# zhaozijie2022/LocoTouch

Hardware: AMD Instinct MI355X
Metric: env-steps/sec (whole node), TransportTeacher 4096 envs/GPU (higher is better)
Workload: dtype f32

## Files before the change

locotouch_amd/_abi.py:

```python
from __future__ import annotations

import ctypes
import os
import re

_HERE = os.path.dirname(os.path.abspath(__file__))
REPO = os.path.dirname(_HERE)
LIB_PATH = os.environ.get("LOCOTOUCH_AMD_LIB", os.path.join(_HERE, "_lib", "liblocotouch_env.so"))

_SCALARS = {"int": ctypes.c_int, "int32_t": ctypes.c_int32, "int64_t": ctypes.c_int64, "uint8_t": ctypes.c_uint8,
            "uint32_t": ctypes.c_uint32, "uint64_t": ctypes.c_uint64, "size_t": ctypes.c_size_t, "float": ctypes.c_float,
            "double": ctypes.c_double}
_DECL = re.compile(r"(?:const\s+)?(\w+)\s*((?:\*\s*(?:const\b\s*)?)*)(\w*)\s*((?:\[[^\]]*\]\s*)*)")


def _ctype(decl, structs, opaque, consts, typed, param):
    m = _DECL.fullmatch(decl.strip())
    if not m:
        return None
    base, stars, name, dims = m.groups()
    depth = stars.count("*")
    try:
        dims = [sum(int(t) if t.strip().isdigit() else consts[t.strip()] for t in d.split("+")) for d in re.findall(r"\[([^\]]*)\]", dims)]
    except KeyError:
# ... 45 lines not shown
        if not m:
            if stmt == "}":
                continue
            raise ImportError(f"cannot parse declaration {stmt!r}")
        ret, name, args = m.groups()
        res = (None, None) if ret.strip() == "void" else _ctype(ret, structs, opaque, consts, typed, param=False)
        args = [] if args.strip() == "void" else [_ctype(a, structs, opaque, consts, typed, param=True) for a in args.split(",")]
        if res is None or None in args:
            raise ImportError(f"cannot type prototype {name}: {' '.join(stmt.split())!r}")
        protos[name] = (res[1], [t for _, t in args])
    return consts, structs, protos


class _CfgMethods(ctypes.Structure):
    def copy(self) -> "LtCfg":
        new = LtCfg()
        ctypes.memmove(ctypes.byref(new), ctypes.byref(self), ctypes.sizeof(self))
        for attr in ("extra_reward_terms", "extra_termination_terms", "extra_observation_terms", "reward_term_params"):
            if hasattr(self, attr):
                v = getattr(self, attr)
                setattr(new, attr, dict(v) if isinstance(v, dict) else list(v))
        return new

    def to_dict(self) -> dict:
        def py(v):
            return [py(x) for x in v] if hasattr(v, "__len__") else v

        return {name: py(getattr(self, name)) for name, *_ in self._fields_ if not name.startswith("_")}


_ENV_VALUE_QUERIES = (
    "lt_abi_version", "lt_cfg_sizeof", "lt_cfg_num_presets", "lt_cfg_preset_id", "lt_cfg_obs_dim", "lt_cfg_tactile_dim", "lt_last_error",
    "lt_wgrad_splits", "lt_wgrad_ws_floats", "lt_elu_backward_bias_ws_floats", "lt_head_wgrad_ws_floats", "lt_adam_clip_step_ws_floats",
    "lt_elu_backward_bias_nblk", "lt_head_wgrad_nblk", "lt_mlp_backward_blocks", "lt_env_kernel_name", "lt_mlp_kernel_name")

HEADERS = (
    ("", "lt_env.h", False, _ENV_VALUE_QUERIES, ("lt_cfg", "lt_view", "lt_mlp_desc", "lt_render_view", "lt_render_desc")),
    ("OBS_NORM", "lt_obs_norm.h", False, (), ()),
    ("STUDENT", "lt_student.h", True, ("lt_student_step_launches",), ("lt_student_desc", "lt_student_params")),
    ("COLLECT", "lt_collect.h", False, (), ()),
    ("LEDGER", "lt_ledger.h", False, (), ()),
    ("CNN_TRAIN", "lt_cnn_train.h", False, ("lt_cnn_launches",), ("lt_cnn_desc", "lt_cnn_params", "lt_cnn_grads")),
    ("BC", "lt_bc.h", False, (), ()),
    ("LSTM", "lt_lstm.h", False, (), ()),
    ("MEMORY", "lt_memory.h", False, (), ("lt_memory_net",)),
    ("MEMORY_SEQ", "lt_memory_seq.h", False, ("lt_memory_seq_backward_units",), ("lt_memory_seq_net", "lt_memory_seq_grad")),
    ("MEMORY_GRU", "lt_memory_gru.h", False, ("lt_memory_gru_seq_backward_units",),
     ("lt_memory_gru_net", "lt_memory_gru_seq_net", "lt_memory_gru_seq_grad")),
    ("POLICY", "lt_policy.h", True, ("lt_policy_step_launches",), ("lt_policy_desc", "lt_policy_memory")),
    ("PPO_OPTS", "lt_ppo_opts.h", False, (), ()),
    ("MLP_DX", "lt_mlp_dx.h", True, (), ()),
    ("PPO_SYM", "lt_ppo_sym.h", False, (), ()),
    ("ENCODER", "lt_encoder.h", False, ("lt_encoder_forward_launches",), ("lt_encoder_desc", "lt_encoder_net")),
)


def _bind(table, include_dir):
    bound, seen, env_structs = [], set(), None
    for prefix, fname, uses_env_structs, queries, _ in table:
        path, queries = os.path.join(include_dir, fname), frozenset(queries)
        consts, structs, sigs = parse_header(open(path).read(), structs=env_structs if uses_env_structs else None, bases={"lt_cfg": _CfgMethods})
        if not prefix:
            env_structs = structs
        for name in sorted(queries - set(sigs)):
            raise ImportError(f"include/{fname}: the value query {name} named in _abi.HEADERS is not declared there")
        for name, (restype, _) in sigs.items():
            if name in seen:
                raise ImportError(f"include/{fname}: {name} repeats an entry point of an earlier header")
            if restype is not ctypes.c_int and (prefix or name not in queries):
                raise ImportError(f"include/{fname}: {name} returns no int (a new value query of lt_env.h belongs in _abi.HEADERS)")
        seen.update(sigs)
        bound.append((path, consts, structs, sigs, queries))
    return bound


ALL_SIGNATURES: dict = {}
ALL_VALUE_QUERIES: set = set()
for (_prefix, _, _, _, _published), (_path, _consts, _structs, _sigs, _queries) in zip(HEADERS, _bind(HEADERS, os.path.join(REPO, "include"))):
    _p = _prefix + "_" if _prefix else ""
    globals().update(_consts)
    globals().update({_p + "HEADER": _path, _p + "CONSTS": _consts, _p + "SIGNATURES": _sigs, _p + "VALUE_QUERIES": _queries})
    globals().update({_structs[_c].__name__: _structs[_c] for _c in _published})
    if not _prefix:
        STRUCTS, EXPORTS = _structs, list(_sigs)
    ALL_SIGNATURES.update(_sigs)
    ALL_VALUE_QUERIES |= _queries

_lib = None
_calls: dict = {}


def load() -> ctypes.CDLL:
    global _lib
    if _lib is not None:
        return _lib
    if not os.path.exists(LIB_PATH):
        raise ImportError(f"{LIB_PATH} is missing: run `python -c 'import __graft_entry__ as g; g.build()'` "
                          "(the HIP extension is mandatory, there is no CPU fallback)")
    lib = ctypes.CDLL(LIB_PATH)
    for name, (restype, argtypes) in ALL_SIGNATURES.items():
        fn = getattr(lib, name)
        fn.restype, fn.argtypes = restype, argtypes
        if name not in ALL_VALUE_QUERIES:
            _calls[name] = (fn, [ptr if t is ctypes.c_void_p else _ref if issubclass(t, ctypes._Pointer) and issubclass(t._type_, ctypes.Structure)
                                 else None for t in argtypes])
    if lib.lt_cfg_sizeof() != ctypes.sizeof(LtCfg):
# ... 77 lines not shown
```

locotouch_amd/csrc/lt_ppo.hip:

```cpp
#include <hip/hip_runtime.h>
#include <math.h>
#include <stdint.h>

#include "lt_env.h"
#include "lt_host_check.h"
#include "lt_internal.h"
#include "lt_ppo_device.h"

namespace {

template <bool LOG, bool NORM>
__global__ __launch_bounds__(256) void lt_ppo_loss_kernel(const float* __restrict__ mu, const float* __restrict__ stdp, const float* __restrict__ value,
                                                          const float* __restrict__ actions, const float* __restrict__ old_logp,
                                                          const float* __restrict__ adv, const float* __restrict__ returns,
                                                          const float* __restrict__ old_values, const float* __restrict__ old_mu,
                                                          const float* __restrict__ old_sigma, const long long* __restrict__ idx,
                                                          long long M, int A, float clip, float vcoef, int clipped_value,
                                                          const float* __restrict__ adv_stats, float* __restrict__ dmu, float* __restrict__ dvalue, float* __restrict__ acc) {
  const long long row = (long long)blockIdx.x * 256 + threadIdx.x;
  const bool ok = row < M;
  const long long src = (ok && idx) ? idx[row] : row;
  __shared__ float sigma_lds[MAX_A];
  if constexpr (LOG) {
    if ((int)threadIdx.x < A) sigma_lds[threadIdx.x] = lt_sigma_of_log(stdp[threadIdx.x]);
    __syncthreads();
  }
  float part[4 + MAX_A];
  float amax_mu = 0.f, amax_v = 0.f;
#pragma unroll
  for (int i = 0; i < 4 + MAX_A; ++i) part[i] = 0.f;
  if (ok) {
    const float inv_m = 1.f / (float)M;
    float logp = 0.f, kl = 0.f;
    float z[MAX_A], isg[MAX_A];
#pragma unroll
    for (int a = 0; a < MAX_A; ++a) {
      if (a < A) {
        const float sg = LOG ? sigma_lds[a] : stdp[a], m = mu[row * A + a], x = actions[src * A + a];
        const float om = old_mu[src * A + a], os = old_sigma[src * A + a];
        isg[a] = 1.f / sg;
        z[a] = (x - m) * isg[a];
        logp += lt_ppo_logp_term<LOG>(z[a], sg, stdp[a]);
        kl += lt_ppo_kl_term(sg, os, om, m);
      }
    }
    float advr = adv[src];
    if constexpr (NORM) advr = (advr - adv_stats[0]) * adv_stats[1];
    const float ratio = __expf(logp - old_logp[src]);
    LT_PPO_SURROGATE(advr, ratio, clip, s1, s2, dsurr_dratio)
    const float dlogp = dsurr_dratio * ratio * inv_m;
#pragma unroll
    for (int a = 0; a < MAX_A; ++a) {
      if (a < A) {
        dmu[row * A + a] = dlogp * z[a] * isg[a];
        amax_mu = fmaxf(amax_mu, fabsf(dlogp * z[a] * isg[a]));
        if constexpr (LOG) part[4 + a] = dlogp * (z[a] * z[a] - 1.f);
        else part[4 + a] = dlogp * (z[a] * z[a] - 1.f) * isg[a];
      }
    }
    const float v = value[row], R = returns[src];
// ... 269 lines not shown
    p[i] = pi - step_size * (mi / (sqrtf(vi) / bc2_sqrt + eps));
  }
}

__global__ __launch_bounds__(64) void lt_std_from_log_kernel(const float* __restrict__ log_std, int A, float* __restrict__ stdp) {
  if ((int)threadIdx.x < A) stdp[threadIdx.x] = lt_sigma_of_log(log_std[threadIdx.x]);
}

__device__ __forceinline__ double lt_block_sum_f64(double v, double* red) {
#pragma unroll
  for (int off = 32; off > 0; off >>= 1) v += __shfl_xor(v, off, 64);
  __syncthreads();
  if ((threadIdx.x & 63) == 0) red[threadIdx.x >> 6] = v;
  __syncthreads();
  return (red[0] + red[1]) + (red[2] + red[3]);
}

__global__ __launch_bounds__(256) void lt_adv_stats_kernel(const float* __restrict__ adv, const long long* __restrict__ idx, long long M,
                                                           float* __restrict__ stats) {
#pragma clang fp reciprocal(off)
  __shared__ double red[4];
  const long long base = (long long)blockIdx.x * M;
  double s = 0.0;
  for (long long r = threadIdx.x; r < M; r += 256) s += (double)adv[idx ? idx[base + r] : base + r];
  const double mean = lt_block_sum_f64(s, red) / (double)M;
  double q = 0.0;
  for (long long r = threadIdx.x; r < M; r += 256) {
    const double d = (double)adv[idx ? idx[base + r] : base + r] - mean;
    q += d * d;
  }
  const double var = lt_block_sum_f64(q, red) / (double)(M - 1);
  if (threadIdx.x == 0) {
    stats[2 * blockIdx.x] = (float)mean;
    stats[2 * blockIdx.x + 1] = (float)(1.0 / (sqrt(var) + (double)1.0e-8f));
  }
}

__global__ __launch_bounds__(64) void lt_ppo_lr_rule_kernel(const float* __restrict__ kl_mean, float desired, float lr_min, float lr_max, float factor,
                                                            float* __restrict__ lr, float* __restrict__ stats, const float* __restrict__ scalars,
                                                            float* __restrict__ dstd_out, int A) {
  if (dstd_out && scalars && (int)threadIdx.x < A) dstd_out[threadIdx.x] = scalars[8 + threadIdx.x];
  if (threadIdx.x != 0) return;
  if (kl_mean && desired > 0.f) {
#pragma clang fp reciprocal(off)
    const float kl = *kl_mean;
    float v = *lr;
    if (kl > desired * 2.f) v = fmaxf(lr_min, v / factor);
    else if (kl < desired * 0.5f && kl > 0.f) v = fminf(lr_max, v * factor);
    *lr = v;
  }
  if (stats && scalars) { stats[0] += scalars[2]; stats[1] += scalars[1]; stats[2] += scalars[3]; }
}

}

extern "C" int lt_ppo_lr_rule(const float* kl_mean, float desired_kl, float lr_min, float lr_max, float factor, float* lr, float* stats,
                              const float* scalars, float* dstd_out, int num_actions, void* stream) {
  if (!lr || factor <= 1.f || num_actions < 0 || num_actions > MAX_A) return einval("lt_ppo_lr_rule: invalid argument");
  hipLaunchKernelGGL(lt_ppo_lr_rule_kernel, dim3(1), dim3(64), 0, (hipStream_t)stream, kl_mean, desired_kl, lr_min, lr_max, factor, lr, stats, scalars,
                     dstd_out, num_actions);
  return launch_status();
}

static int elu_backward_bias(const float* da, const float* a, int64_t M, int N, float alpha, float* dz, float* db, float* ws, float* amax, void* stream);
extern "C" int lt_elu_backward_bias(const float* da, const float* a, int64_t M, int N, float alpha, float* dz, float* db, float* ws, void* stream) {
  return elu_backward_bias(da, a, M, N, alpha, dz, db, ws, nullptr, stream);
}
extern "C" int lt_elu_backward_bias2(const float* da, const float* a, int64_t M, int N, float alpha, float* dz, float* db, float* ws, float* amax_blocks,
                                     void* stream) {
  return elu_backward_bias(da, a, M, N, alpha, dz, db, ws, amax_blocks, stream);
}
static int elu_backward_bias(const float* da, const float* a, int64_t M, int N, float alpha, float* dz, float* db, float* ws, float* amax, void* stream) {
  if (!da || !a || !dz || !ws || M < 1 || N < 4 || (N & 3) || N > 1024)
    return einval("lt_elu_backward_bias: invalid argument (N a multiple of 4, 4 <= N <= 1024)");
  const int nblk = (int)((M + EB_ROWS - 1) / EB_ROWS);
  hipLaunchKernelGGL(lt_elu_bwd_bias_kernel, dim3((unsigned)nblk), dim3(256), 0, (hipStream_t)stream, da, a, (long long)M, N, alpha, dz, ws, amax);
  if (db) launch_one_sum(ws, nblk, (long long)N, N, N, db, nullptr, (hipStream_t)stream);
  return launch_status();
}

extern "C" int64_t lt_head_wgrad_ws_floats(int64_t M, int n, int k) { return ((M + HW_ROWS - 1) / HW_ROWS) * ((int64_t)n * k + HW_MAX_N); }

extern "C" int lt_head_wgrad(const float* dy, const float* x, int x_split, int64_t M, int n, int k, float* dw, float* db, float* ws, void* stream) {
  if (!dy || !x || !ws || M < 1 || n < 1 || n > HW_MAX_N || k < 4 || (k & 3) || k > 1024)
    return einval("lt_head_wgrad: invalid argument (1 <= n <= 16, k a multiple of 4, 4 <= k <= 1024)");
  const int nblk = (int)((M + HW_ROWS - 1) / HW_ROWS), k4 = k / 4, lanes = 256 / k4;
  const int nn = n <= 1 ? 1 : (n <= 4 ? 4 : (n <= 8 ? 8 : (n <= 12 ? 12 : 16)));
  const size_t lds = (size_t)lanes * nn * k4 * 16 + (size_t)lanes * nn * 4;
  if (const int e = lt_ensure_dynamic_lds((const void*)lt_head_wgrad_kernel<16>, 72 * 1024)) {
    lt_set_error(hipGetErrorString((hipError_t)e));
    return LT_EHIP;
  }
  if (lds > 72 * 1024) return einval("lt_head_wgrad: n * k too large for one block's LDS partials");
  const dim3 g((unsigned)nblk), b(256);
  hipStream_t st = (hipStream_t)stream;
  switch (nn) {
    case 1: hipLaunchKernelGGL(lt_head_wgrad_kernel<1>, g, b, lds, st, dy, x, x_split, (long long)M, n, k, ws); break;
    case 4: hipLaunchKernelGGL(lt_head_wgrad_kernel<4>, g, b, lds, st, dy, x, x_split, (long long)M, n, k, ws); break;
    case 8: hipLaunchKernelGGL(lt_head_wgrad_kernel<8>, g, b, lds, st, dy, x, x_split, (long long)M, n, k, ws); break;
    case 12: hipLaunchKernelGGL(lt_head_wgrad_kernel<12>, g, b, lds, st, dy, x, x_split, (long long)M, n, k, ws); break;
    default: hipLaunchKernelGGL(lt_head_wgrad_kernel<16>, g, b, lds, st, dy, x, x_split, (long long)M, n, k, ws); break;
  }
  if (dw) launch_one_sum(ws, nblk, (long long)n * k + HW_MAX_N, n * k + n, n * k, dw, db, st);
  return launch_status();
}

// ... 77 lines not shown
                       std_is_log ? 1 : 0, out);
  return launch_status();
}

extern "C" int lt_ppo_loss(const float* mu, const float* stdp, const float* value, const float* actions, const float* old_logp, const float* adv,
                           const float* returns, const float* old_values, const float* old_mu, const float* old_sigma, const int64_t* idx,
                           int64_t M, int A, float clip, float value_loss_coef, float entropy_coef, int use_clipped_value_loss, float* dmu, float* dvalue,
                           float* acc, float* out, void* stream) {
  if (!mu || !stdp || !value || !actions || !old_logp || !adv || !returns || !old_values || !old_mu || !old_sigma || !dmu || !dvalue || !acc ||
      M < 1 || A < 1 || A > MAX_A)
    return einval("lt_ppo_loss: invalid argument (1 <= num_actions <= 16)");
  return ppo_loss(mu, stdp, value, actions, old_logp, adv, returns, old_values, old_mu, old_sigma, idx, M, A, clip, value_loss_coef,
                  entropy_coef, use_clipped_value_loss, 0, nullptr, dmu, dvalue, acc, out, stream);
}

extern "C" int lt_ppo_loss_opts(const float* mu, const float* stdp, const float* value, const float* actions, const float* old_logp,
                                const float* adv, const float* returns, const float* old_values, const float* old_mu, const float* old_sigma,
                                const int64_t* idx, int64_t M, int A, float clip, float value_loss_coef, float entropy_coef,
                                int use_clipped_value_loss, int std_is_log, const float* adv_stats, float* dmu, float* dvalue, float* acc,
                                float* out, void* stream) {
  const char* fn = "lt_ppo_loss_opts";
  const ptr_check ptrs[] = {{"mu", mu, 4}, {"std", stdp, 4}, {"value", value, 4}, {"actions", actions, 4}, {"old_logp", old_logp, 4}, {"adv", adv, 4},
                            {"returns", returns, 4}, {"old_values", old_values, 4}, {"old_mu", old_mu, 4}, {"old_sigma", old_sigma, 4},
                            {"dmu", dmu, 4}, {"dvalue", dvalue, 4}, {"acc", acc, 4}};
  if (const int rc = check_ptrs(fn, "", ptrs)) return rc;
  if ((uintptr_t)idx % 8 != 0) return refuse(fn, "", "idx", "NULL or 8-byte aligned");
  if ((uintptr_t)adv_stats % 4 != 0) return refuse(fn, "", "adv_stats", "NULL or 4-byte aligned");
  if ((uintptr_t)out % 4 != 0) return refuse(fn, "", "out", "NULL or 4-byte aligned");
  if (M < 1) return refuse(fn, "", "M", ">= 1");
  if (A < 1 || A > MAX_A) return refuse(fn, "", "A", "in [1, 16]");
  return ppo_loss(mu, stdp, value, actions, old_logp, adv, returns, old_values, old_mu, old_sigma, idx, M, A, clip, value_loss_coef, entropy_coef,
                  use_clipped_value_loss, std_is_log, adv_stats, dmu, dvalue, acc, out, stream);
}

extern "C" int lt_std_from_log(const float* log_std, int A, float* stdp, void* stream) {
  const char* fn = "lt_std_from_log";
  const ptr_check ptrs[] = {{"log_std", log_std, 4}, {"std", stdp, 4}};
  if (const int rc = check_ptrs(fn, "", ptrs)) return rc;
  if (A < 1 || A > MAX_A) return refuse(fn, "", "A", "in [1, 16]");
  hipLaunchKernelGGL(lt_std_from_log_kernel, dim3(1), dim3(64), 0, (hipStream_t)stream, log_std, A, stdp);
  return launch_status();
}

extern "C" int lt_adv_stats(const float* adv, const int64_t* idx, int64_t M, int nmb, float* stats, void* stream) {
  const char* fn = "lt_adv_stats";
  const ptr_check ptrs[] = {{"adv", adv, 4}, {"stats", stats, 4}};
  if (const int rc = check_ptrs(fn, "", ptrs)) return rc;
  if ((uintptr_t)idx % 8 != 0) return refuse(fn, "", "idx", "NULL or 8-byte aligned");
  if (M < 2) return refuse(fn, "", "M", ">= 2 (the unbiased std of one element is NaN)");
  if (nmb < 1) return refuse(fn, "", "nmb", ">= 1");
  hipLaunchKernelGGL(lt_adv_stats_kernel, dim3((unsigned)nmb), dim3(256), 0, (hipStream_t)stream, adv, (const long long*)idx, (long long)M, stats);
  return launch_status();
}
```

locotouch_amd/rl/flat_adam.py:

```python
from __future__ import annotations

import torch

from .. import _abi


class FlatAdam:
    ALIGN = 64

    def __init__(self, optimizer: torch.optim.Adam):
        if type(optimizer) is not torch.optim.Adam or len(optimizer.param_groups) != 1:
            raise TypeError("FlatAdam wraps a single-group torch.optim.Adam")
        g = optimizer.param_groups[0]
        if g.get("amsgrad") or g.get("maximize") or g.get("capturable") or g.get("differentiable"):
            raise TypeError("FlatAdam: amsgrad / maximize / capturable / differentiable are not supported")
        self.optimizer = optimizer
        self.params = [p for p in g["params"] if p.requires_grad]
        if not self.params or any(p.dtype != torch.float32 or not p.is_cuda for p in self.params):
            raise TypeError("FlatAdam needs f32 CUDA parameters")
        self.offsets, off = [], 0
        for p in self.params:
            self.offsets.append(off)
            off += -(-p.numel() // self.ALIGN) * self.ALIGN
        self.n = off
# ... 18 lines not shown
                    v.copy_(p.data)
                    p.data = v
            self._gviews = [v for _, v in self._views(self.flat_g)]
            steps = {float(st[p]["step"]) for p in self.params if p in st and "step" in st[p]}
            if len(steps) > 1:
                raise ValueError("FlatAdam: the parameters' Adam step counts differ")
            self.step_count = int(steps.pop()) if steps else 0
            for name, flat in (("exp_avg", self.flat_m), ("exp_avg_sq", self.flat_v)):
                for p, v in self._views(flat):
                    s = st[p]
                    if name not in s:
                        v.zero_()
                    elif s[name].data_ptr() != v.data_ptr():
                        v.copy_(s[name])
                    s[name] = v
            self._step_t = torch.tensor(float(self.step_count))
            for p in self.params:
                st[p]["step"] = self._step_t

    def _bound(self) -> bool:
        p0 = self.params[0]
        s0 = self.optimizer.state.get(p0, {})
        return (p0.data.data_ptr() == self.flat_p.data_ptr() and "exp_avg" in s0 and s0["exp_avg"].data_ptr() == self.flat_m.data_ptr()
                and s0.get("step") is self._step_t)

    def zero_grad(self) -> None:
        for p in self.params:
            p.grad = None

    def gather_grads(self) -> torch.Tensor:
        have = [(v, p.grad) for p, v in zip(self.params, self._gviews) if p.grad is not None and p.grad.data_ptr() != v.data_ptr()]
        missing = [v for p, v in zip(self.params, self._gviews) if p.grad is None]
        if have:
            torch._foreach_copy_([v for v, _ in have], [g for _, g in have])
        if missing:
            torch._foreach_zero_(missing)
        for p, v in zip(self.params, self._gviews):
            p.grad = v
        return self.flat_g

    def grad_views(self) -> dict:
        if not self._bound():
            self._adopt()
        for p, v in zip(self.params, self._gviews):
            p.grad = v
        return {p: v for p, v in zip(self.params, self._gviews)}

    def offset_of(self, param) -> int:
        for p, off in zip(self.params, self.offsets):
            if p is param:
                return off
        raise KeyError("parameter not in the flat bucket")

    def step_dev(self, max_norm: float, lr_dev: torch.Tensor) -> None:
        if not self._bound():
            self._adopt()
        g = self.optimizer.param_groups[0]
        self.step_count += 1
        b1, b2 = g["betas"]
        _abi.call("lt_adam_clip_step_dev", self.flat_p, self.flat_g, self.flat_m, self.flat_v, self.n, float(max_norm or 0.0), lr_dev,
                  float(b1), float(b2), float(g["eps"]), float(g["weight_decay"]), self.step_count, self._ws, self.grad_norm,
                  _abi.stream(self.flat_p.device))
        self._step_t.fill_(float(self.step_count))

    def step(self, max_norm: float, gathered: bool = False) -> None:
        if not self._bound():
            self._adopt()
        if not gathered:
            self.gather_grads()
        g = self.optimizer.param_groups[0]
        self.step_count += 1
        b1, b2 = g["betas"]
        _abi.call("lt_adam_clip_step", self.flat_p, self.flat_g, self.flat_m, self.flat_v, self.n, float(max_norm or 0.0), float(g["lr"]),
                  float(b1), float(b2), float(g["eps"]), float(g["weight_decay"]), self.step_count, self._ws, self.grad_norm,
                  _abi.stream(self.flat_p.device))
        self._step_t.fill_(float(self.step_count))
```

locotouch_amd/rl/ppo.py:

```python
from __future__ import annotations

import torch
import torch.nn as nn

from .. import _abi
from .dist import Dist
from .modules import ActorCritic
from .storage import RolloutStorage


class PPO:
    def __init__(self, actor_critic: ActorCritic, num_learning_epochs=1, num_mini_batches=1, clip_param=0.2, gamma=0.998,
                 lam=0.95, value_loss_coef=1.0, entropy_coef=0.0, learning_rate=1e-3, max_grad_norm=1.0,
                 use_clipped_value_loss=True, schedule="fixed", desired_kl=0.01, device="cpu",
                 normalize_advantage_per_mini_batch=False, dist: Dist | None = None, rnd_cfg: dict | None = None,
                 symmetry_cfg: dict | None = None, **unused):
        if rnd_cfg is not None:
            raise NotImplementedError("rnd_cfg: random network distillation is not built (DESIGN.md §7: it needs an `rnd_state` observation "
                                      "group no env here produces); pass rnd_cfg=None")
        self.symmetry = self._resolve_symmetry(symmetry_cfg, actor_critic)
        self._sym_tables = None
        self.device = device
        self.dist = dist or Dist()
        self.actor_critic = actor_critic.to(device)
        on_gpu = torch.device(device).type == "cuda"
        self.fused_loss = on_gpu and bool(unused.get("fused_loss", True))
        self.packed_forward = on_gpu and bool(unused.get("packed_forward", True))
        self.direct_update = on_gpu and bool(unused.get("direct_update", True))
        self.fused_recurrent_update = bool(unused.get("fused_recurrent_update", False))
        self.fused_gru_memories = bool(unused.get("fused_gru_memories", False))
        self.direct_recurrent_update = bool(unused.get("direct_recurrent_update", False))
        self.fused_encoder_policy = bool(unused.get("fused_encoder_policy", False))
        self._encoders = None
        if self.fused_encoder_policy:
            if self.fused_recurrent_update or self.direct_recurrent_update or self.fused_gru_memories:
                raise ValueError("fused_encoder_policy: the recurrent keys (fused_recurrent_update, direct_recurrent_update, fused_gru_memories) "
                                 "belong to ActorCriticRecurrent: an encoder policy has no memories")
            if self.symmetry is not None:
                raise ValueError("fused_encoder_policy: symmetry_cfg is not served for an encoder policy (the mirror tables cover the plain ActorCritic's rows)")
            if self.dist.world_size > 1:
                raise ValueError(f"fused_encoder_policy: dist.world_size is {self.dist.world_size}: the collectives of this form are not "
                                 "covered by a multi-rank test, it runs on one rank only")
            if not on_gpu:
                raise ValueError(f"fused_encoder_policy: the device is {device!r}: its kernels run on a GPU only")
        if self.direct_recurrent_update:
            if not self.fused_recurrent_update:
                raise ValueError("direct_recurrent_update: it is a form of the whole-rollout update: set fused_recurrent_update=True as well")
            if not on_gpu:
                raise ValueError(f"direct_recurrent_update: the device is {device!r}: its kernels run on a GPU only")
            if self.dist.world_size > 1:
                raise ValueError(f"direct_recurrent_update: dist.world_size is {self.dist.world_size}: the collectives of this form are not "
                                 "covered by a multi-rank test, it runs on one rank only")
            why = self._recurrent_update_unsupported()
            if why is not None:
                raise ValueError(f"direct_recurrent_update: {why}")
        if self.fused_recurrent_update:
            why = self._recurrent_update_unsupported()
            if why is not None:
                raise ValueError(f"fused_recurrent_update: {why}")
        self._pair = None
        if on_gpu and bool(unused.get("tuned_gemms", True)):
            from . import tuned_gemms

            tuned_gemms.enable()
        self.optimizer = torch.optim.Adam(self.actor_critic.parameters(), lr=learning_rate)
        self.storage: RolloutStorage | None = None
        self.learning_rate = learning_rate
        self.schedule, self.desired_kl = schedule, desired_kl
        self.clip_param, self.gamma, self.lam = clip_param, gamma, lam
        self.num_learning_epochs, self.num_mini_batches = num_learning_epochs, num_mini_batches
        self.value_loss_coef, self.entropy_coef, self.max_grad_norm = value_loss_coef, entropy_coef, max_grad_norm
        self.use_clipped_value_loss = use_clipped_value_loss
        self.normalize_advantage_per_mini_batch = normalize_advantage_per_mini_batch
        self._t = {}
        self._flat_grad: torch.Tensor | None = None
        self._flat_adam = None
        use_flat_adam = on_gpu and bool(unused.get("fused_adam", True))
        if self.dist.world_size > 1:
            if not use_flat_adam:
                self._make_flat_grad_bucket()
            self.broadcast_parameters()
# ... 122 lines not shown
        obs, cobs, small = self._flat_storage()
        stats = torch.zeros(3, device=obs.device)
        pair = self._packed_pair()
        std_p, std_is_log = std_param(ac)
        if pair is not None and self._flat_adam is not None and self.direct_update and std_p.requires_grad:
            return self._direct_update(pair)
        if pair is not None:
            pair.arm_domain_check()
        perm, mb = st.mini_batch_permutation(self.num_mini_batches)
        mb_stats = adv_stats(small[2], perm, mb, self.num_mini_batches) if self.normalize_advantage_per_mini_batch else None
        for step_i in range(self.num_learning_epochs * self.num_mini_batches):
            i = step_i % self.num_mini_batches
            idx = perm[i * mb:(i + 1) * mb]
            o, co = obs[idx], cobs[idx]
            if o.dtype != torch.float32:
                o, co = o.float(), co.float()
            mu, value = pair(o, co) if pair is not None else (ac.actor(o), ac.critic(co))
            loss, surrogate_loss, value_loss, ent, kl_mean = fused_ppo_loss(
                mu, std_p, value, *small, self.clip_param, self.value_loss_coef, self.entropy_coef,
                self.use_clipped_value_loss, idx=idx, std_is_log=std_is_log, adv_stats=None if mb_stats is None else mb_stats[i])
            kl_handle = self.dist.all_reduce_mean_begin(kl_mean.detach().clone()) if self._adaptive else None
            self._zero_grad()
            loss.backward()
            if self._adaptive:
                self._apply_kl(self.dist.all_reduce_mean_end(kl_handle), reduced=True)
            self._optim_step()
            stats = stats + torch.stack((value_loss, surrogate_loss, ent.detach()))
        n = self.num_learning_epochs * self.num_mini_batches
        sv, ss, se = (stats / n).tolist()
        if pair is not None and pair.domain_violated():
            self._warn_mlp_domain()
        st.clear()
        return sv, ss, se, None, None

    def _direct_update(self, pair, split_buckets: bool = True):
        ac, fa, sym = self.actor_critic, self._flat_adam, self.symmetry
        perm, m = self.storage.mini_batch_permutation(self.num_mini_batches)
        c = self._direct_begin("direct_update", pair, perm, m, symmetric=sym is not None)
        obs, cobs, dev, grad_of = c.obs, c.cobs, c.dev, c.grad_of
        critic_at = fa.offset_of(next(iter(ac.critic.parameters())))
        two_buckets = split_buckets and 0 < critic_at < self._flat_grad.numel()
        sym_args = None
        if sym is None:
            rows = m
            perm_o, perm_co = obs[perm], cobs[perm]
            if perm_o.dtype != torch.float32:
                perm_o, perm_co = perm_o.float(), perm_co.float()
        else:
            rows = 2 * m
            tab_o, tab_co, tab_a = self._symmetry_tables(dev, obs.shape[1], cobs.shape[1], c.a_dim)
            perm_o, perm_co = (self._symmetry_gather(x, perm, m, t) for x, t in ((obs, tab_o), (cobs, tab_co)))
            sym_args = (tab_a, float(sym["mirror_loss_coeff"]) if sym["use_mirror_loss"] else 0.0)
        split_o = (pair.split_rows(perm_o), pair.split_rows(perm_co)) if pair._fused_backward_possible(perm_o[:rows], perm_co[:rows]) else None
        for step_i in range(self.num_learning_epochs * self.num_mini_batches):
            i = step_i % self.num_mini_batches
            idx = perm[i * m:(i + 1) * m]
            o, co = perm_o[i * rows:(i + 1) * rows], perm_co[i * rows:(i + 1) * rows]
            xs = (split_o[0][i * rows:(i + 1) * rows], split_o[1][i * rows:(i + 1) * rows]) if split_o is not None else None
            (mu, value), acts = pair.forward_raw(o, co)
            dmu, dvalue, acc = self._direct_loss_and_rule(c, mu, value, idx, m, i, sym_args)
            if self.dist.world_size > 1 and two_buckets:
                handles = []
                pair.backward_raw(o, co, acts, dmu, dvalue, grad_of, xs, after_first=lambda: handles.append(self.dist.all_reduce_mean_begin(self._flat_grad[:critic_at])),
                                  dy_amax=(acc[20:21], acc[21:22]))
                handles.append(self.dist.all_reduce_mean_begin(self._flat_grad[critic_at:] if handles else self._flat_grad))
                for h in handles:
                    self.dist.all_reduce_mean_end(h)
            else:
                pair.backward_raw(o, co, acts, dmu, dvalue, grad_of, xs, dy_amax=(acc[20:21], acc[21:22]))
                if self.dist.world_size > 1:
                    self.dist.all_reduce_mean_(self._flat_grad)
            fa.step_dev(self.max_grad_norm, c.lr_dev)
        return self._direct_end(c, with_dx=False)

    def _direct_begin(self, key: str, pair, index, m: int, symmetric: bool = False):
        from types import SimpleNamespace

        from .fused_loss import adv_stats, std_param

        obs, cobs, small = self._flat_storage()
        small = [t.view(-1) if t.shape[-1] == 1 else t for t in small]
        a_dim = small[0].shape[1]
        if a_dim > 16:
            raise ValueError(f"{key}: the action width is {a_dim}: the loss kernel serves at most 16")
        dev = obs.device
        state = torch.zeros(5 if symmetric else 4, device=dev)
        state[0] = self.learning_rate
        std_p, std_is_log = std_param(self.actor_critic)
        pair.arm_domain_check()
        mb_stats = adv_stats(small[2], index, m, self.num_mini_batches) if self.normalize_advantage_per_mini_batch else None
        return SimpleNamespace(pair=pair, obs=obs, cobs=cobs, small=small, a_dim=a_dim, dev=dev, state=state, lr_dev=state[:1], stats=state[1:4],
                               grad_of=self._flat_adam.grad_views(), std_p=std_p, std_is_log=std_is_log, std_c=std_p.detach(),
                               stream=_abi.stream(dev), mb_stats=mb_stats)

    def _direct_loss_and_rule(self, c, mu, value, idx, m: int, i: int, sym_args=None):
        dev = c.dev
        dmu = torch.empty_like(mu)
        dvalue = torch.empty(mu.shape[0], 1, device=dev, dtype=torch.float32)
        acc = torch.empty(24, device=dev, dtype=torch.float32)
        out = torch.empty(24, device=dev, dtype=torch.float32)
        rows = (mu, c.std_c, value, *c.small, idx, m, c.a_dim, float(self.clip_param), float(self.value_loss_coef), float(self.entropy_coef),
                int(bool(self.use_clipped_value_loss)))
        opts = (int(c.std_is_log), None if c.mb_stats is None else c.mb_stats[i])
        if sym_args is not None:
            _abi.call("lt_ppo_loss_sym", *rows, *opts, *sym_args, dmu, dvalue, acc, out, c.state[4:5], c.stream)
        elif c.std_is_log or c.mb_stats is not None:
            _abi.call("lt_ppo_loss_opts", *rows, *opts, dmu, dvalue, acc, out, c.stream)
        else:
            _abi.call("lt_ppo_loss", *rows, dmu, dvalue, acc, out, c.stream)
        kl = None
        if self._adaptive:
            kl = out[4:5]
            if self.dist.world_size > 1:
                kl = self.dist.all_reduce_mean_(kl.clone())
        _abi.call("lt_ppo_lr_rule", kl, float(self.desired_kl or 0.0), 1e-5, 1e-2, 1.5, c.lr_dev, c.stats, out, c.grad_of[c.std_p], c.a_dim, c.stream)
        return dmu, dvalue, acc

    def _direct_end(self, c, with_dx: bool):
        pair, state = c.pair, c.state
        sat, dom = pair.saturated(), pair.domain_max
        pair.domain_max = None
        zero = state.new_zeros(1)
        read = torch.cat((state, zero if sat is None else sat, zero if dom is None else dom.view(1))).tolist()
        (lr, sv, ss, se), (nsat, dmax) = read[:4], read[-2:]
        if nsat > 0:
            import warnings

            sat.zero_()
            entry = "lt_mlp_backward_pair_dx" if with_dx and pair._dx_kernel_ok() else "lt_mlp_backward_pair"
            warnings.warn(f"{entry}: {int(nsat)} workgroup-layers of the gradient chain reached the f16 image's bound "
                          "(a gradient grew by more than 500x through the layers): those rows were saturated; set LT_FUSED_BACKWARD=0 "
                          "to run the chain as f32 library GEMMs")
        self.learning_rate = lr
        for group in self.optimizer.param_groups:
            group["lr"] = lr
        if dmax >= float(_abi.CONSTS["LT_MLP_INPUT_CLAMP"]):
            self._warn_mlp_domain()
        self.storage.clear()
        n = self.num_learning_epochs * self.num_mini_batches
        return sv / n, ss / n, se / n, None, read[4] / n if state.numel() == 5 else None

    def _symmetry_tables(self, dev, obs_dim: int, critic_obs_dim: int, a_dim: int):
        if self._sym_tables is None:
            from .symmetry import mirror_tables

            tables = mirror_tables(self.symmetry["_env"])
            packed = []
            for kind, width in (("policy", obs_dim), ("critic", critic_obs_dim), ("action", a_dim)):
                src, sign = tables.of(kind)
                if src.numel() != width:
                    raise ValueError(f"symmetry_cfg: the env's {kind} mirror table covers {src.numel()} columns, the storage's rows have {width}")
                buf = torch.empty(width, device=dev, dtype=torch.int32)
                _abi.call("lt_sym_table_pack", src.contiguous(), sign.contiguous(), width, buf, _abi.stream(dev))
# ... 432 lines not shown
```

Measured before the change: 68.75 million.

## Pre-gather PPO minibatch rows once and use row-tiled loss and vectorised Adam

Before the update epochs, one kernel gathers the per-sample PPO inputs (actions, old mu/sigma, logp, adv, returns, values) into contiguous padded records, so each minibatch's loss kernel reads coalesced float4 rows instead of indirect per-field gathers. The new loss kernel stages a 128-row tile in LDS and splits the action dimension across 4 lanes per row. A separate finalize kernel merges the loss finalization and the LR rule, and a float4-vectorised Adam kernel moves the step-count fill out of the loop to a single sync after it. The cost is an extra buffer of M×W floats and a one-time gather, and the path only applies to the single-GPU, non-symmetric, non-log-std case.

New measurement: 68.55 million, median of 2. No clear change (-0.3%).

```diff
diff --git a/include/lt_ppo_step.h b/include/lt_ppo_step.h
--- /dev/null
+++ b/include/lt_ppo_step.h
@@ -0,0 +1,31 @@
+#ifndef LT_PPO_STEP_H
+#define LT_PPO_STEP_H
+
+#include <stddef.h>
+#include <stdint.h>
+
+#ifdef __cplusplus
+extern "C" {
+#endif
+
+int lt_ppo_row_floats(int A);
+
+int lt_ppo_gather_rows(const float* actions, const float* old_logp, const float* adv, const float* returns, const float* old_values,
+                       const float* old_mu, const float* old_sigma, const int64_t* idx, int64_t M_total, int A, float* rows_out,
+                       void* stream);
+
+int lt_ppo_loss_rows(const float* mu, const float* std, const float* value, const float* rows, int64_t M, int A, float clip,
+                     float value_loss_coef, int use_clipped_value_loss, float* dmu, float* dvalue, float* acc, void* stream);
+
+int lt_ppo_finalize_rule(const float* acc, const float* std, int A, int64_t M, float value_loss_coef, float entropy_coef, int adaptive,
+                         float desired_kl, float lr_min, float lr_max, float factor, float* lr, float* stats, float* out, float* dstd_out,
+                         void* stream);
+
+int lt_adam_clip_step_dev4(float* params, float* grads, float* exp_avg, float* exp_avg_sq, int64_t n, float max_norm, const float* lr_dev,
+                           float beta1, float beta2, float eps, float weight_decay, int64_t step, float* ws, float* grad_norm, void* stream);
+
+#ifdef __cplusplus
+}
+#endif
+
+#endif
diff --git a/locotouch_amd/_abi.py b/locotouch_amd/_abi.py
--- a/locotouch_amd/_abi.py
+++ b/locotouch_amd/_abi.py
@@ -121,6 +121,7 @@
     ("MLP_DX", "lt_mlp_dx.h", True, (), ()),
     ("PPO_SYM", "lt_ppo_sym.h", False, (), ()),
     ("ENCODER", "lt_encoder.h", False, ("lt_encoder_forward_launches",), ("lt_encoder_desc", "lt_encoder_net")),
+    ("PPO_STEP", "lt_ppo_step.h", False, ("lt_ppo_row_floats",), ()),
 )
 
 
diff --git a/locotouch_amd/csrc/lt_ppo.hip b/locotouch_amd/csrc/lt_ppo.hip
--- a/locotouch_amd/csrc/lt_ppo.hip
+++ b/locotouch_amd/csrc/lt_ppo.hip
@@ -6,6 +6,7 @@
 #include "lt_host_check.h"
 #include "lt_internal.h"
 #include "lt_ppo_device.h"
+#include "lt_ppo_step.h"
 
 namespace {
 
@@ -381,6 +382,254 @@
   if (stats && scalars) { stats[0] += scalars[2]; stats[1] += scalars[1]; stats[2] += scalars[3]; }
 }
 
+__host__ __device__ constexpr int lt_row_floats(int A) { return (3 * A + 4 + 3) & ~3; }
+
+__global__ __launch_bounds__(256) void lt_ppo_gather_rows_kernel(const float* __restrict__ actions, const float* __restrict__ old_logp,
+                                                                 const float* __restrict__ adv, const float* __restrict__ returns,
+                                                                 const float* __restrict__ old_values, const float* __restrict__ old_mu,
+                                                                 const float* __restrict__ old_sigma, const long long* __restrict__ idx,
+                                                                 long long M, int A, float* __restrict__ rows_out) {
+  const int W = lt_row_floats(A);
+  const long long e = (long long)blockIdx.x * 256 + threadIdx.x;
+  if (e >= M * W) return;
+  const long long r = e / W;
+  const int c = (int)(e - r * W);
+  const long long src = idx ? idx[r] : r;
+  float v = 0.f;
+  if (c < A) v = actions[src * A + c];
+  else if (c < 2 * A) v = old_mu[src * A + (c - A)];
+  else if (c < 3 * A) v = old_sigma[src * A + (c - 2 * A)];
+  else if (c == 3 * A) v = old_logp[src];
+  else if (c == 3 * A + 1) v = adv[src];
+  else if (c == 3 * A + 2) v = returns[src];
+  else if (c == 3 * A + 3) v = old_values[src];
+  rows_out[e] = v;
+}
+
+constexpr int LR_ROWS = 128;
+constexpr int LR_LANES = 4;
+constexpr int LR_THREADS = LR_ROWS * LR_LANES;
+constexpr int LR_SLOTS = MAX_A / LR_LANES;
+constexpr int LR_PASSES = LR_ROWS * 16 / LR_THREADS;
+
+__global__ __launch_bounds__(LR_THREADS) void lt_ppo_loss_rows_kernel(const float* __restrict__ mu, const float* __restrict__ stdp,
+                                                                       const float* __restrict__ value, const float* __restrict__ rows,
+                                                                       long long M, int A, float clip, float vcoef, int clipped_value,
+                                                                       float* __restrict__ dmu, float* __restrict__ dvalue, float* __restrict__ acc) {
+  constexpr int MAX_W = lt_row_floats(MAX_A);
+  __shared__ float rec_lds[LR_ROWS * (MAX_W + 1)];
+  __shared__ float mu_lds[LR_ROWS * (MAX_A + 1)];
+  const int W = lt_row_floats(A), ws = W + 1, as = A | 1;
+  const long long r0 = (long long)blockIdx.x * LR_ROWS;
+  const int nrows = (int)((M - r0) < LR_ROWS ? (M - r0) : LR_ROWS);
+  const int tr = (int)threadIdx.x / LR_LANES, q = (int)threadIdx.x % LR_LANES;
+  const long long row = r0 + tr;
+  const bool ok = tr < nrows;
+  const int sr = (int)threadIdx.x >> 4, sc = (int)threadIdx.x & 15;
+  const bool mu4 = (A & 3) == 0;
+  const float v = (ok && q == 0) ? value[row] : 0.f;
+  float4 rv[LR_PASSES], mv[LR_PASSES];
+#pragma unroll
+  for (int k = 0; k < LR_PASSES; ++k) {
+    const int r = sr + k * (LR_THREADS / 16);
+    if (r < nrows && 4 * sc < W) rv[k] = ((const float4*)(rows + (r0 + r) * W))[sc];
+    if (mu4) {
+      if (r < nrows && 4 * sc < A) mv[k] = ((const float4*)(mu + (r0 + r) * A))[sc];
+    } else if (r < nrows && sc < A) {
+      mv[k].x = mu[(r0 + r) * A + sc];
+    }
+  }
+#pragma unroll
+  for (int k = 0; k < LR_PASSES; ++k) {
+    const int r = sr + k * (LR_THREADS / 16);
+    if (r < nrows && 4 * sc < W) {
+      float* const d = rec_lds + r * ws + 4 * sc;
+      d[0] = rv[k].x; d[1] = rv[k].y; d[2] = rv[k].z; d[3] = rv[k].w;
+    }
+    if (mu4) {
+      if (r < nrows && 4 * sc < A) {
+        float* const d = mu_lds + r * as + 4 * sc;
+        d[0] = mv[k].x; d[1] = mv[k].y; d[2] = mv[k].z; d[3] = mv[k].w;
+      }
+    } else if (r < nrows && sc < A) {
+      mu_lds[r * as + sc] = mv[k].x;
+    }
+  }
+  __syncthreads();
+  const float* const rec = rec_lds + tr * ws;
+  float* const mrow = mu_lds + tr * as;
+  float z[LR_SLOTS], isg[LR_SLOTS], t_logp[LR_SLOTS], t_kl[LR_SLOTS];
+#pragma unroll
+  for (int j = 0; j < LR_SLOTS; ++j) {
+    const int a = q + j * LR_LANES;
+    z[j] = isg[j] = t_logp[j] = t_kl[j] = 0.f;
+    if (ok && a < A) {
+      const float sg = stdp[a], m = mrow[a], x = rec[a];
+      const float om = rec[A + a], os = rec[2 * A + a];
+      isg[j] = 1.f / sg;
+      z[j] = (x - m) * isg[j];
+      t_logp[j] = lt_ppo_logp_term<false>(z[j], sg, stdp[a]);
+      t_kl[j] = lt_ppo_kl_term(sg, os, om, m);
+    }
+  }
+  float logp = 0.f, kl = 0.f;
+  const int lane0 = (int)(threadIdx.x & 63) & ~(LR_LANES - 1);
+#pragma unroll
+  for (int a = 0; a < MAX_A; ++a) {
+    if (a < A) {
+      logp += __shfl(t_logp[a / LR_LANES], lane0 + a % LR_LANES, 64);
+      kl += __shfl(t_kl[a / LR_LANES], lane0 + a % LR_LANES, 64);
+    }
+  }
+  float dsg[LR_SLOTS], rowsum[3] = {0.f, 0.f, 0.f};
+  float amax_mu = 0.f, amax_v = 0.f;
+#pragma unroll
+  for (int j = 0; j < LR_SLOTS; ++j) dsg[j] = 0.f;
+  if (ok) {
+    const float inv_m = 1.f / (float)M;
+    const float advr = rec[3 * A + 1];
+    const float ratio = __expf(logp - rec[3 * A]);
+    LT_PPO_SURROGATE(advr, ratio, clip, s1, s2, dsurr_dratio)
+    const float dlogp = dsurr_dratio * ratio * inv_m;
+#pragma unroll
+    for (int j = 0; j < LR_SLOTS; ++j) {
+      const int a = q + j * LR_LANES;
+      if (a < A) {
+        mrow[a] = dlogp * z[j] * isg[j];
+        amax_mu = fmaxf(amax_mu, fabsf(dlogp * z[j] * isg[j]));
+        dsg[j] = dlogp * (z[j] * z[j] - 1.f) * isg[j];
+      }
+    }
+    if (q == 0) {
+      const float R = rec[3 * A + 2];
+      float vl, dv;
+      LT_PPO_VALUE_LOSS(v, R, rec, 3 * A + 3, clip, clipped_value, vl, dv)
+      dvalue[row] = vcoef * dv * inv_m;
+      amax_v = fabsf(vcoef * dv * inv_m);
+      rowsum[0] = fmaxf(s1, s2);
+      rowsum[1] = vl;
+      rowsum[2] = kl;
+    }
+  }
+  __syncthreads();
+#pragma unroll
+  for (int k = 0; k < LR_PASSES; ++k) {
+    const int r = sr + k * (LR_THREADS / 16);
+    if (mu4) {
+      if (r < nrows && 4 * sc < A) {
+        const float* const d = mu_lds + r * as + 4 * sc;
+        ((float4*)(dmu + (r0 + r) * A))[sc] = make_float4(d[0], d[1], d[2], d[3]);
+      }
+    } else if (r < nrows && sc < A) {
+      dmu[(r0 + r) * A + sc] = mu_lds[r * as + sc];
+    }
+  }
+  constexpr int NW = LR_THREADS / 64;
+  __shared__ float red[NW][4 + MAX_A];
+  __shared__ float redm[NW][2];
+  const int lane = threadIdx.x & 63, wave = threadIdx.x >> 6;
+#pragma unroll
+  for (int off = 32; off >= LR_LANES; off >>= 1) {
+#pragma unroll
+    for (int j = 0; j < LR_SLOTS; ++j) dsg[j] += __shfl_xor(dsg[j], off, 64);
+#pragma unroll
+    for (int i = 0; i < 3; ++i) rowsum[i] += __shfl_xor(rowsum[i], off, 64);
+  }
+#pragma unroll
+  for (int off = 32; off > 0; off >>= 1) {
+    amax_mu = fmaxf(amax_mu, __shfl_xor(amax_mu, off, 64));
+    amax_v = fmaxf(amax_v, __shfl_xor(amax_v, off, 64));
+  }
+  if (lane < LR_LANES) {
+#pragma unroll
+    for (int j = 0; j < LR_SLOTS; ++j) red[wave][4 + lane + j * LR_LANES] = dsg[j];
+  }
+  if (lane == 0) {
+    red[wave][0] = rowsum[0]; red[wave][1] = rowsum[1]; red[wave][2] = rowsum[2];
+    redm[wave][0] = amax_mu; redm[wave][1] = amax_v;
+  }
+  __syncthreads();
+  if ((int)threadIdx.x < 4 + A && threadIdx.x != 3) {
+    float s = red[0][threadIdx.x];
+#pragma unroll
+    for (int w = 1; w < NW; ++w) s += red[w][threadIdx.x];
+    atomicAdd(acc + threadIdx.x, s);
+  } else if (threadIdx.x >= 64 && threadIdx.x < 66) {
+    const int j = threadIdx.x - 64;
+    float mx = redm[0][j];
+#pragma unroll
+    for (int w = 1; w < NW; ++w) mx = fmaxf(mx, redm[w][j]);
+    atomicMax((unsigned*)acc + 20 + j, __float_as_uint(mx));
+  }
+}
+
+__global__ __launch_bounds__(64) void lt_ppo_finalize_rule_kernel(const float* __restrict__ acc, const float* __restrict__ stdp, int A, float inv_m,
+                                                                  float vcoef, float ecoef, int adaptive, float desired, float lr_min, float lr_max,
+                                                                  float factor, float* __restrict__ lr, float* __restrict__ stats, float* out,
+                                                                  float* __restrict__ dstd_out) {
+  lt_ppo_finalize(acc, stdp, A, inv_m, vcoef, ecoef, 0, out);
+  __syncthreads();
+  if (dstd_out && (int)threadIdx.x < A) dstd_out[threadIdx.x] = out[8 + threadIdx.x];
+  if (threadIdx.x != 0) return;
+  if (adaptive && desired > 0.f) {
+#pragma clang fp reciprocal(off)
+    const float kl = out[4];
+    float v = *lr;
+    if (kl > desired * 2.f) v = fmaxf(lr_min, v / factor);
+    else if (kl < desired * 0.5f && kl > 0.f) v = fminf(lr_max, v * factor);
+    *lr = v;
+  }
+  if (stats) { stats[0] += out[2]; stats[1] += out[1]; stats[2] += out[3]; }
+}
+
+__device__ __forceinline__ void lt_adam_element(float& p, float& g, float& m, float& v, float coef, float b1, float b2, float eps, float wd,
+                                                float step_size, float inv_bc2_sqrt) {
+  const float pi = p;
+  const float gi = fmaf(coef, g, wd * pi);
+  g = g * coef;
+  const float mi = fmaf(1.f - b1, gi - m, m);
+  const float vi = fmaf(b2, v, ((1.f - b2) * gi) * gi);
+  m = mi;
+  v = vi;
+  p = fmaf(-step_size, __builtin_amdgcn_rcpf(fmaf(sqrtf(vi), inv_bc2_sqrt, eps)) * mi, pi);
+}
+
+__global__ __launch_bounds__(256) void lt_adam4_kernel(float* __restrict__ p, float* __restrict__ g, float* __restrict__ m, float* __restrict__ v,
+                                                       long long n, const float* __restrict__ ws, int nblk, float max_norm, float b1, float b2,
+                                                       float eps, float wd, float bc2_sqrt, float* __restrict__ norm_out,
+                                                       const float* __restrict__ lr_dev, float inv_bc1) {
+  __shared__ float s_coef;
+  const float step_size = *lr_dev * inv_bc1;
+  if (threadIdx.x < 64) {
+    float s = 0.f;
+    for (int b = threadIdx.x; b < nblk; b += 64) s += ws[b];
+    for (int off = 32; off > 0; off >>= 1) s += __shfl_xor(s, off, 64);
+    if (threadIdx.x == 0) {
+      const float norm = sqrtf(s);
+      const float c = max_norm / (norm + 1.0e-6f);
+      s_coef = max_norm > 0.f ? (c < 1.f ? c : 1.f) : 1.f;
+      if (blockIdx.x == 0 && norm_out) *norm_out = norm;
+    }
+  }
+  __syncthreads();
+  const float coef = s_coef, inv_bc2_sqrt = __builtin_amdgcn_rcpf(bc2_sqrt);
+  const long long base = (long long)blockIdx.x * AD_PER_BLOCK;
+#pragma unroll
+  for (int u = 0; u < AD_PER_BLOCK / 1024; ++u) {
+    const long long i = base + u * 1024 + 4 * (int)threadIdx.x;
+    if (i + 3 < n) {
+      float4 P = *(float4*)(p + i), G = *(float4*)(g + i), Mo = *(float4*)(m + i), V = *(float4*)(v + i);
+      lt_adam_element(P.x, G.x, Mo.x, V.x, coef, b1, b2, eps, wd, step_size, inv_bc2_sqrt);
+      lt_adam_element(P.y, G.y, Mo.y, V.y, coef, b1, b2, eps, wd, step_size, inv_bc2_sqrt);
+      lt_adam_element(P.z, G.z, Mo.z, V.z, coef, b1, b2, eps, wd, step_size, inv_bc2_sqrt);
+      lt_adam_element(P.w, G.w, Mo.w, V.w, coef, b1, b2, eps, wd, step_size, inv_bc2_sqrt);
+      *(float4*)(g + i) = G; *(float4*)(m + i) = Mo; *(float4*)(v + i) = V; *(float4*)(p + i) = P;
+    } else {
+      for (long long j = i; j < n && j < i + 4; ++j) lt_adam_element(p[j], g[j], m[j], v[j], coef, b1, b2, eps, wd, step_size, inv_bc2_sqrt);
+    }
+  }
+}
+
 }
 
 extern "C" int lt_ppo_lr_rule(const float* kl_mean, float desired_kl, float lr_min, float lr_max, float factor, float* lr, float* stats,
@@ -564,3 +813,66 @@
   hipLaunchKernelGGL(lt_adv_stats_kernel, dim3((unsigned)nmb), dim3(256), 0, (hipStream_t)stream, adv, (const long long*)idx, (long long)M, stats);
   return launch_status();
 }
+
+extern "C" int lt_ppo_row_floats(int A) { return lt_row_floats(A); }
+
+extern "C" int lt_ppo_gather_rows(const float* actions, const float* old_logp, const float* adv, const float* returns, const float* old_values,
+                                  const float* old_mu, const float* old_sigma, const int64_t* idx, int64_t M_total, int A, float* rows_out,
+                                  void* stream) {
+  const char* fn = "lt_ppo_gather_rows";
+  const ptr_check ptrs[] = {{"actions", actions, 4}, {"old_logp", old_logp, 4}, {"adv", adv, 4}, {"returns", returns, 4}, {"old_values", old_values, 4},
+                            {"old_mu", old_mu, 4}, {"old_sigma", old_sigma, 4}, {"rows_out", rows_out, 16}};
+  if (const int rc = check_ptrs(fn, "", ptrs)) return rc;
+  if ((uintptr_t)idx % 8 != 0) return refuse(fn, "", "idx", "NULL or 8-byte aligned");
+  if (A < 1 || A > MAX_A) return refuse(fn, "", "A", "in [1, 16]");
+  if (M_total < 1 || M_total > (int64_t)0x7fffffff * 256 / lt_row_floats(A)) return refuse(fn, "", "M_total", ">= 1 and within one launch's grid");
+  const long long total = (long long)M_total * lt_row_floats(A);
+  hipLaunchKernelGGL(lt_ppo_gather_rows_kernel, dim3((unsigned)((total + 255) / 256)), dim3(256), 0, (hipStream_t)stream, actions, old_logp, adv, returns,
+                     old_values, old_mu, old_sigma, (const long long*)idx, (long long)M_total, A, rows_out);
+  return launch_status(fn);
+}
+
+extern "C" int lt_ppo_loss_rows(const float* mu, const float* stdp, const float* value, const float* rows, int64_t M, int A, float clip,
+                                float value_loss_coef, int use_clipped_value_loss, float* dmu, float* dvalue, float* acc, void* stream) {
+  const char* fn = "lt_ppo_loss_rows";
+  const ptr_check ptrs[] = {{"mu", mu, 16}, {"std", stdp, 4}, {"value", value, 4}, {"rows", rows, 16}, {"dmu", dmu, 16}, {"dvalue", dvalue, 4}, {"acc", acc, 4}};
+  if (const int rc = check_ptrs(fn, "", ptrs)) return rc;
+  if (A < 1 || A > MAX_A) return refuse(fn, "", "A", "in [1, 16]");
+  if (M < 1 || M > (int64_t)0x7fffffff * LR_ROWS) return refuse(fn, "", "M", ">= 1 and within one launch's grid");
+  hipLaunchKernelGGL(lt_ppo_loss_rows_kernel, dim3((unsigned)((M + LR_ROWS - 1) / LR_ROWS)), dim3(LR_THREADS), 0, (hipStream_t)stream, mu, stdp, value, rows,
+                     (long long)M, A, clip, value_loss_coef, use_clipped_value_loss, dmu, dvalue, acc);
+  return launch_status(fn);
+}
+
+extern "C" int lt_ppo_finalize_rule(const float* acc, const float* stdp, int A, int64_t M, float value_loss_coef, float entropy_coef, int adaptive,
+                                    float desired_kl, float lr_min, float lr_max, float factor, float* lr, float* stats, float* out, float* dstd_out,
+                                    void* stream) {
+  const char* fn = "lt_ppo_finalize_rule";
+  const ptr_check ptrs[] = {{"acc", acc, 4}, {"std", stdp, 4}, {"lr", lr, 4}, {"out", out, 4}};
+  if (const int rc = check_ptrs(fn, "", ptrs)) return rc;
+  if ((uintptr_t)stats % 4 != 0) return refuse(fn, "", "stats", "NULL or 4-byte aligned");
+  if ((uintptr_t)dstd_out % 4 != 0) return refuse(fn, "", "dstd_out", "NULL or 4-byte aligned");
+  if (A < 1 || A > MAX_A) return refuse(fn, "", "A", "in [1, 16]");
+  if (M < 1) return refuse(fn, "", "M", ">= 1");
+  if (!(factor > 1.f)) return refuse(fn, "", "factor", "> 1");
+  hipLaunchKernelGGL(lt_ppo_finalize_rule_kernel, dim3(1), dim3(64), 0, (hipStream_t)stream, acc, stdp, A, 1.f / (float)M, value_loss_coef, entropy_coef,
+                     adaptive, desired_kl, lr_min, lr_max, factor, lr, stats, out, dstd_out);
+  return launch_status(fn);
+}
+
+extern "C" int lt_adam_clip_step_dev4(float* params, float* grads, float* exp_avg, float* exp_avg_sq, int64_t n, float max_norm, const float* lr_dev,
+                                      float beta1, float beta2, float eps, float weight_decay, int64_t step, float* ws, float* grad_norm, void* stream) {
+  const char* fn = "lt_adam_clip_step_dev4";
+  const ptr_check ptrs[] = {{"params", params, 16}, {"grads", grads, 16}, {"exp_avg", exp_avg, 16}, {"exp_avg_sq", exp_avg_sq, 16}, {"lr_dev", lr_dev, 4},
+                            {"ws", ws, 4}};
+  if (const int rc = check_ptrs(fn, "", ptrs)) return rc;
+  if ((uintptr_t)grad_norm % 4 != 0) return refuse(fn, "", "grad_norm", "NULL or 4-byte aligned");
+  if (n < 1) return refuse(fn, "", "n", ">= 1");
+  if (step < 1) return refuse(fn, "", "step", ">= 1");
+  const int nblk = (int)((n + AD_PER_BLOCK - 1) / AD_PER_BLOCK);
+  const double bc1 = 1.0 - pow((double)beta1, (double)step), bc2 = 1.0 - pow((double)beta2, (double)step);
+  hipLaunchKernelGGL(lt_sumsq_kernel, dim3((unsigned)nblk), dim3(256), 0, (hipStream_t)stream, grads, (long long)n, ws);
+  hipLaunchKernelGGL(lt_adam4_kernel, dim3((unsigned)nblk), dim3(256), 0, (hipStream_t)stream, params, grads, exp_avg, exp_avg_sq, (long long)n, ws, nblk,
+                     max_norm, beta1, beta2, eps, weight_decay, (float)sqrt(bc2), grad_norm, lr_dev, (float)(1.0 / bc1));
+  return launch_status(fn);
+}
diff --git a/locotouch_amd/rl/flat_adam.py b/locotouch_amd/rl/flat_adam.py
--- a/locotouch_amd/rl/flat_adam.py
+++ b/locotouch_amd/rl/flat_adam.py
@@ -94,15 +94,19 @@
                 return off
         raise KeyError("parameter not in the flat bucket")
 
-    def step_dev(self, max_norm: float, lr_dev: torch.Tensor) -> None:
+    def step_dev(self, max_norm: float, lr_dev: torch.Tensor, vec4: bool = False) -> None:
         if not self._bound():
             self._adopt()
         g = self.optimizer.param_groups[0]
         self.step_count += 1
         b1, b2 = g["betas"]
-        _abi.call("lt_adam_clip_step_dev", self.flat_p, self.flat_g, self.flat_m, self.flat_v, self.n, float(max_norm or 0.0), lr_dev,
-                  float(b1), float(b2), float(g["eps"]), float(g["weight_decay"]), self.step_count, self._ws, self.grad_norm,
-                  _abi.stream(self.flat_p.device))
+        _abi.call("lt_adam_clip_step_dev4" if vec4 else "lt_adam_clip_step_dev", self.flat_p, self.flat_g, self.flat_m, self.flat_v, self.n,
+                  float(max_norm or 0.0), lr_dev, float(b1), float(b2), float(g["eps"]), float(g["weight_decay"]), self.step_count, self._ws,
+                  self.grad_norm, _abi.stream(self.flat_p.device))
+        if not vec4:
+            self._step_t.fill_(float(self.step_count))
+
+    def sync_step(self) -> None:
         self._step_t.fill_(float(self.step_count))
 
     def step(self, max_norm: float, gathered: bool = False) -> None:
diff --git a/locotouch_amd/rl/ppo.py b/locotouch_amd/rl/ppo.py
--- a/locotouch_amd/rl/ppo.py
+++ b/locotouch_amd/rl/ppo.py
@@ -27,6 +27,7 @@
         self.fused_loss = on_gpu and bool(unused.get("fused_loss", True))
         self.packed_forward = on_gpu and bool(unused.get("packed_forward", True))
         self.direct_update = on_gpu and bool(unused.get("direct_update", True))
+        self.direct_step_kernels = bool(unused.get("direct_step_kernels", True))
         self.fused_recurrent_update = bool(unused.get("fused_recurrent_update", False))
         self.fused_gru_memories = bool(unused.get("fused_gru_memories", False))
         self.direct_recurrent_update = bool(unused.get("direct_recurrent_update", False))
@@ -255,13 +256,20 @@
             perm_o, perm_co = (self._symmetry_gather(x, perm, m, t) for x, t in ((obs, tab_o), (cobs, tab_co)))
             sym_args = (tab_a, float(sym["mirror_loss_coeff"]) if sym["use_mirror_loss"] else 0.0)
         split_o = (pair.split_rows(perm_o), pair.split_rows(perm_co)) if pair._fused_backward_possible(perm_o[:rows], perm_co[:rows]) else None
-        for step_i in range(self.num_learning_epochs * self.num_mini_batches):
+        steps = self.num_learning_epochs * self.num_mini_batches
+        step_kernels = (self.direct_step_kernels and sym is None and not c.std_is_log and c.mb_stats is None and self.dist.world_size == 1)
+        if step_kernels:
+            records = torch.empty(perm.numel(), _abi.load().lt_ppo_row_floats(c.a_dim), device=dev, dtype=torch.float32)
+            _abi.call("lt_ppo_gather_rows", *c.small, perm, perm.numel(), c.a_dim, records, c.stream)
+            accs = torch.zeros(steps, 24, device=dev, dtype=torch.float32)
+        for step_i in range(steps):
             i = step_i % self.num_mini_batches
             idx = perm[i * m:(i + 1) * m]
             o, co = perm_o[i * rows:(i + 1) * rows], perm_co[i * rows:(i + 1) * rows]
             xs = (split_o[0][i * rows:(i + 1) * rows], split_o[1][i * rows:(i + 1) * rows]) if split_o is not None else None
             (mu, value), acts = pair.forward_raw(o, co)
-            dmu, dvalue, acc = self._direct_loss_and_rule(c, mu, value, idx, m, i, sym_args)
+            dmu, dvalue, acc = self._direct_loss_and_rule(c, mu, value, idx, m, i, sym_args,
+                                                          records=(records[i * m:(i + 1) * m], accs[step_i]) if step_kernels else None)
             if self.dist.world_size > 1 and two_buckets:
                 handles = []
                 pair.backward_raw(o, co, acts, dmu, dvalue, grad_of, xs, after_first=lambda: handles.append(self.dist.all_reduce_mean_begin(self._flat_grad[:critic_at])),
@@ -273,7 +281,9 @@
                 pair.backward_raw(o, co, acts, dmu, dvalue, grad_of, xs, dy_amax=(acc[20:21], acc[21:22]))
                 if self.dist.world_size > 1:
                     self.dist.all_reduce_mean_(self._flat_grad)
-            fa.step_dev(self.max_grad_norm, c.lr_dev)
+            fa.step_dev(self.max_grad_norm, c.lr_dev, vec4=step_kernels)
+        if step_kernels:
+            fa.sync_step()
         return self._direct_end(c, with_dx=False)
 
     def _direct_begin(self, key: str, pair, index, m: int, symmetric: bool = False):
@@ -296,12 +306,19 @@
                                grad_of=self._flat_adam.grad_views(), std_p=std_p, std_is_log=std_is_log, std_c=std_p.detach(),
                                stream=_abi.stream(dev), mb_stats=mb_stats)
 
-    def _direct_loss_and_rule(self, c, mu, value, idx, m: int, i: int, sym_args=None):
+    def _direct_loss_and_rule(self, c, mu, value, idx, m: int, i: int, sym_args=None, records=None):
         dev = c.dev
         dmu = torch.empty_like(mu)
         dvalue = torch.empty(mu.shape[0], 1, device=dev, dtype=torch.float32)
+        out = torch.empty(24, device=dev, dtype=torch.float32)
+        if records is not None:
+            rec, acc = records
+            _abi.call("lt_ppo_loss_rows", mu, c.std_c, value, rec, m, c.a_dim, float(self.clip_param), float(self.value_loss_coef),
+                      int(bool(self.use_clipped_value_loss)), dmu, dvalue, acc, c.stream)
+            _abi.call("lt_ppo_finalize_rule", acc, c.std_c, c.a_dim, m, float(self.value_loss_coef), float(self.entropy_coef), int(self._adaptive),
+                      float(self.desired_kl or 0.0), 1e-5, 1e-2, 1.5, c.lr_dev, c.stats, out, c.grad_of[c.std_p], c.stream)
+            return dmu, dvalue, acc
         acc = torch.empty(24, device=dev, dtype=torch.float32)
-        out = torch.empty(24, device=dev, dtype=torch.float32)
         rows = (mu, c.std_c, value, *c.small, idx, m, c.a_dim, float(self.clip_param), float(self.value_loss_coef), float(self.entropy_coef),
                 int(bool(self.use_clipped_value_loss)))
         opts = (int(c.std_is_log), None if c.mb_stats is None else c.mb_stats[i])
```
